# david-zwicker/video-analysis

Measured on AMD Instinct MI355X. Metric: frames/sec (bg-sub+blur+thresh+CCL) 1080p uint8, higher is better.
Workload: dtype u8; 1 GPU; cfg3_1080p_full_chain: 1920x1080 uint8, batch 256/GPU, running-mean bg-sub (f64 state) + sigma=5 Gaussian (q8.8) + threshold 20 + 5x5 dilate/erode + 4-connected labelling + object counts; inputs resident in HBM; engine=bg=1 gauss=mfma-i8(ksize=31) thresh=20 morph=2 ccl=4, video=one clip per rank, overlap=off, world_size=1, backend=single process

## Files before the change

### video-analysis_amd/csrc/va_api.hip

```cpp
#include <dlfcn.h>
#include <stdarg.h>
#include <stdlib.h>

#include <mutex>
#include <vector>
#include <new>

#include "va_common.h"

namespace va {

static thread_local char g_err[512] = "";

void set_error(const char *fmt, ...)
{
    va_list ap;
    va_start(ap, fmt);
    vsnprintf(g_err, sizeof(g_err), fmt, ap);
    va_end(ap);
}
const char *get_error() { return g_err; }

struct ScratchBlock {
    void *ptr;
// ... 108 lines not shown
    void *blur;
    void *gscratch;
    int planes_wp;
    uint32_t *bits[2][2];
    void *ccl_ws[2];
    size_t ccl_ws_bytes;
    size_t bits_bytes;
    bool overlap;
    int slot;
    hipStream_t side;
    int paint_grid;
    hipEvent_t ev_front;
    hipEvent_t ev_paint[2];
    bool paint_pending[2];
    const char *paint_lo[2], *paint_hi[2];
    const char *pstat_lo[2], *pstat_hi[2];
    int32_t *labels_scratch;
    int32_t *counts_scratch;
    TapsQ8 tq;
    TapsF32 tf;
    RowSpans se[VA_MAX_MORPH_OPS];
    bool fused;
    bool mfma;
    bool f32_fused;
    char desc[160];
    StageProfiler *prof;
};

template <class T>
static int resize_any(const T *src, T *dst, int n, int src_h, int src_w, int c, int dst_h, int dst_w,
                      int interpolation, void *stream, const char *who)
{
    VA_ENTER();
    VA_REQUIRE(src && dst && src != dst, "%s: src/dst must be distinct non-NULL", who);
    VA_REQUIRE(n >= 0 && src_h > 0 && src_w > 0 && dst_h > 0 && dst_w > 0 && c >= 1 && c <= 4,
               "%s: bad shape (%d,%d,%d,%d) -> (%d,%d)", who, n, src_h, src_w, c, dst_h, dst_w);
    VA_REQUIRE((size_t)src_h * src_w < kMaxFramePixels && (size_t)dst_h * dst_w < kMaxFramePixels,
               "%s: frames above 2^29 pixels are not supported", who);
    VA_REQUIRE(interpolation >= VA_INTER_NEAREST && interpolation <= VA_INTER_LANCZOS4,
               "%s: interpolation %d not supported (0 nearest, 1 linear, 2 cubic, 3 area, 4 lanczos4)", who,
               interpolation);
    ScratchLease scratch;
    int rc = scratch.acquire(resize_scratch_bytes(src_h, src_w, dst_h, dst_w), as_stream(stream));
    if (rc)
        return rc;
    if constexpr (sizeof(T) == 1)
// ... 954 lines not shown
    }
    for (int i = 0; i < cfg->morph_count; i++) {
        if (cfg->morph_op[i] != VA_MORPH_ERODE && cfg->morph_op[i] != VA_MORPH_DILATE) {
            set_error("va_pipeline_create: bad morph_op[%d]=%d", i, cfg->morph_op[i]);
            pipeline_free(p);
            return VA_ERR_INVALID;
        }
        PIPE_TRY(make_row_spans(cfg->morph_shape[i], cfg->morph_ksize[i], &p->se[i]));
    }
    if (cfg->bg_mode != VA_BG_NONE) {
        p->bg_bytes = p->px * (cfg->bg_mode == VA_BG_EMA ? sizeof(float) : sizeof(double));
        PIPE_MALLOC(p->bg_state, p->bg_bytes);
        if (p->f32_fused && cfg->bg_mode == VA_BG_EMA)
            PIPE_MALLOC(p->bg_state_alt, p->bg_bytes);
        p->bg_in_u8_range = true;
        hipError_t e = hipMemset(p->bg_state, 0, p->bg_bytes);
        if (e != hipSuccess) {
            set_error("va_pipeline_create: hipMemset failed: %s", hipGetErrorString(e));
            pipeline_free(p);
            return VA_ERR_HIP;
        }
        if (!p->f32_fused)
            PIPE_MALLOC(p->diff, nb * p->px * esz);
        if (cfg->bg_mode == VA_BG_MEAN)
            PIPE_MALLOC(p->bg_recip, bg_scratch_bytes(cfg->max_batch));
    }
    if (cfg->sigma > 0 && !p->fused) {
        size_t gs = cfg->dtype == VA_U8 ? gauss_generic_u8_scratch_bytes(nb * p->px, p->tq) : nb * p->px * 4;
        if (cfg->dtype == VA_U8) {
            p->planes_wp = planes_width(cfg->height, cfg->width, cfg->channels, p->tq);
            if (p->planes_wp)
                gs = planes_scratch_bytes(cfg->max_batch, cfg->height, p->planes_wp, cfg->channels);
        }
        PIPE_MALLOC(p->gscratch, gs);
        PIPE_MALLOC(p->blur, nb * p->px * esz);
    }
    if (masks) {
        size_t bb = align_up(nb * cfg->height * p->w32 * sizeof(uint32_t));
        p->bits_bytes = bb;
        PIPE_MALLOC(p->bits[0][0], bb);
        PIPE_MALLOC(p->bits[0][1], bb);
        if (cfg->connectivity) {
            p->ccl_ws_bytes = ccl_rows_workspace_bytes(cfg->max_batch, cfg->height);
            PIPE_MALLOC(p->ccl_ws[0], p->ccl_ws_bytes);
            PIPE_MALLOC(p->counts_scratch, align_up(nb * sizeof(int32_t)));
            PIPE_MALLOC(p->labels_scratch, nb * p->frame_px * sizeof(int32_t));
// ... 166 lines not shown
    VA_MARK(nullptr);

    if (c.dtype == VA_F32 && p->f32_fused) {
        VA_REQUIRE(reinterpret_cast<uintptr_t>(frames) % 16 == 0 &&
                       (!filtered_out || reinterpret_cast<uintptr_t>(filtered_out) % 16 == 0),
                   "va_pipeline_run: float32 pipelines need 16-byte aligned frames_dev / filtered_out_dev "
                   "(hipMalloc'ed buffers and whole-frame offsets into them are)");
        void *dst = filtered_out ? filtered_out : p->blur;
        const bool ema = c.bg_mode == VA_BG_EMA;
        rc = launch_gauss_f32_fused((const float *)frames, (float *)dst, (float *)p->gscratch,
                                    ema ? (const float *)p->bg_state : nullptr,
                                    ema ? (float *)p->bg_state_alt : nullptr, p->n_seen, (double)c.bg_rate, n,
                                    c.height, c.width, c.channels, p->tf, st, prof);
        if (rc)
            return rc;
        if (ema && n > 0) {
            std::swap(p->bg_state, p->bg_state_alt);
            p->n_seen += n;
        }
        return VA_OK;
    }
    if (c.bg_mode != VA_BG_NONE) {
        rc = launch_bg(c.bg_mode, c.dtype, cur, p->diff, p->bg_state, p->n_seen, (double)c.bg_rate,
                       n, p->px, st, p->bg_recip, p->bg_in_u8_range);
        if (rc)
            return rc;
        p->n_seen += n;
        cur = p->diff;
        VA_MARK("bg");
    }

    const bool want_ccl = masks && c.connectivity && (labels_out || counts_out || stats_out);
    const bool defer_paint = p->overlap && want_ccl && (labels_out != nullptr || stats_out != nullptr);
    const int slot = defer_paint ? p->slot : 0;
    if (p->overlap && p->paint_pending[slot])
        VA_HIP(hipStreamWaitEvent(st, p->ev_paint[slot], 0));
    uint32_t *const *bits = p->bits[slot];

    bool have_bits = false;
    if (c.sigma > 0) {
        if (c.dtype == VA_U8 && p->mfma && masks && mask_out && !filtered_out && c.morph_count == 0 && !want_ccl &&
            reinterpret_cast<uintptr_t>(mask_out) % 4 == 0) {
            rc = launch_gauss_mfma_u8((const uint8_t *)cur, mask_out, nullptr, c.thresh, n, c.height, c.width, p->tq,
                                      st, c.maxval);
            if (rc)
                return rc;
            VA_MARK("gauss_mfma_mask8");
            return VA_OK;
        }
        if (c.dtype == VA_U8 && p->fused) {
            if (p->mfma)
                rc = launch_gauss_mfma_u8((const uint8_t *)cur, (uint8_t *)filtered_out, masks ? bits[0] : nullptr,
                                          c.thresh, n, c.height, c.width, p->tq, st);
            else
                rc = launch_gauss_fused_u8((const uint8_t *)cur, (uint8_t *)filtered_out, masks ? bits[0] : nullptr,
                                           c.thresh, n, c.height, c.width, p->tq, st);
            if (rc)
                return rc;
            have_bits = masks;
            cur = filtered_out;
            VA_MARK(p->mfma ? "gauss_mfma" : "gauss_fused");
        } else {
            void *dst = filtered_out ? filtered_out : p->blur;
            if (c.dtype == VA_U8 && p->planes_wp)
                rc = blur_u8_planes((const uint8_t *)cur, (uint8_t *)dst, n, c.height, c.width,
                                    p->planes_wp, c.channels, p->tq, p->gscratch, st);
            else if (c.dtype == VA_U8)
                rc = launch_gauss_generic_u8((const uint8_t *)cur, (uint8_t *)dst,
                                             p->gscratch, n, c.height, c.width,
                                             c.channels, p->tq, st);
            else if (gauss_f32_fast_supported(c.width, c.channels, p->tf))
                rc = launch_gauss_f32_fast((const float *)cur, (float *)dst, (float *)p->gscratch, n,
                                           c.height, c.width, c.channels, p->tf, st);
            else
                rc = launch_gauss_generic_f32((const float *)cur, (float *)dst,
                                              (float *)p->gscratch, n, c.height, c.width,
// ... 255 lines not shown
```

### video-analysis_amd/csrc/va_common.h

```cpp
#pragma once
#include <hip/hip_runtime.h>
#include <stdint.h>
#include <stdio.h>
#include <string.h>

#include "../../include/videoanalysis_hip.h"

namespace va {

void set_error(const char *fmt, ...) __attribute__((format(printf, 1, 2)));
const char *get_error();

inline hipStream_t as_stream(void *s) { return reinterpret_cast<hipStream_t>(s); }

#define VA_HIP(call)                                                                        \
    do {                                                                                    \
        hipError_t _e = (call);                                                             \
        if (_e != hipSuccess) {                                                             \
            va::set_error("%s failed: %s (%s:%d)", #call, hipGetErrorString(_e), __FILE__,  \
                          __LINE__);                                                        \
            return _e == hipErrorOutOfMemory ? VA_ERR_NOMEM : VA_ERR_HIP;                   \
        }                                                                                   \
    } while (0)

// ... 65 lines not shown
int launch_gauss_generic_u8(const uint8_t *src, uint8_t *dst, void *scratch, int n, int h,
                            int w, int c, const TapsQ8 &taps, hipStream_t st);
int launch_gauss_generic_f32(const float *src, float *dst, float *scratch, int n, int h, int w,
                             int c, const TapsF32 &taps, hipStream_t st);
bool gauss_f32_fast_supported(int w, int c, const TapsF32 &taps);
int launch_gauss_f32_fast(const float *src, float *dst, float *scratch, int n, int h, int w, int c,
                          const TapsF32 &taps, hipStream_t st);
#if defined(__HIPCC__)
__device__ __forceinline__ void lds_barrier()
{
    asm volatile("s_waitcnt lgkmcnt(0)\n\ts_barrier" ::: "memory");
}
#endif
void gauss_f32_test_hook(int generic_columns);
bool gauss_f32_fused_supported(int h, int w, int c, const TapsF32 &taps);
int launch_gauss_f32_fused(const float *src, float *dst, float *scratch, const float *bg, float *bg_out,
                           int64_t n_seen, double rate, int n, int h, int w, int c, const TapsF32 &taps,
                           hipStream_t st, StageProfiler *prof = nullptr);
bool gauss_fused_supported(int w, int h, const TapsQ8 &taps);
int launch_gauss_fused_u8(const uint8_t *src, uint8_t *dst, uint32_t *bits, int thresh, int n,
                          int h, int w, const TapsQ8 &taps, hipStream_t st);
bool gauss_mfma_supported(int w, int h, const TapsQ8 &taps);
int launch_gauss_mfma_u8(const uint8_t *src, uint8_t *dst, uint32_t *bits, int thresh, int n,
                         int h, int w, const TapsQ8 &taps, hipStream_t st, int mask8_maxval = 0);

size_t bg_scratch_bytes(int n);
int launch_bg(int mode, int dtype, const void *frames, void *diff, void *state, int64_t n_seen,
              double rate, int n, size_t px, hipStream_t st, double *recip_scratch = nullptr,
              bool mean_in_u8_range = false);
int launch_welford(const uint8_t *frames, double *mean, double *m2, int64_t n_seen, int n,
                   size_t px, hipStream_t st);

int launch_temporal_stats(const void *frames, int dtype, double *mean, double *m2, int64_t n_seen, int n,
                          size_t px, hipStream_t st);
int launch_threshold_u8(const uint8_t *src, uint8_t *dst, size_t count, int thresh, int maxval,
                        hipStream_t st);
int launch_time_difference(const uint8_t *a, const uint8_t *b, int16_t *out, size_t count,
                           hipStream_t st);
int launch_mono_mean(const uint8_t *src, uint8_t *dst, size_t pixels, hipStream_t st);
bool launch_pointwise_u8_x4(const uint8_t *src, uint8_t *dst, size_t out_samples, int src_c, int mono, int normalize,
                            double fmin, double fmax, double alpha, double tmin, hipStream_t st);
int launch_channel_planes(const uint8_t *src, uint8_t *dst, int n, int h, int w, int wp, int c,
                          bool split, hipStream_t st);
int launch_rot90(const void *src, void *dst, int n, int h, int w, int elem_bytes, int k,
                 hipStream_t st);
int launch_normalize_u8(const uint8_t *src, uint8_t *dst, size_t count, double fmin, double fmax,
                        double alpha, double tmin, hipStream_t st);

int launch_pack_bits(const uint8_t *src, uint32_t *bits, int n, int h, int w, int thresh,
                     hipStream_t st);
int launch_unpack_bits(const uint32_t *bits, uint8_t *dst, int n, int h, int w, int maxval,
                       hipStream_t st);
// ... 94 lines not shown
```

### video-analysis_amd/csrc/va_gauss_mfma.hip

```cpp
#include "va_common.h"

namespace va {

namespace {

typedef int v4i __attribute__((ext_vector_type(4)));
typedef int v16i __attribute__((ext_vector_type(16)));
typedef uint32_t u4 __attribute__((ext_vector_type(4)));
typedef u4 u4_unaligned __attribute__((aligned(1)));

constexpr int kWaves = 4;
constexpr int kTileCols = kWaves * 32;
constexpr int kLdsStride = kTileCols + 32 + 16;
static_assert((kLdsStride / 16) % 2 == 1, "LDS row stride must be an odd multiple of 16 bytes");
constexpr int kTapTable = 128;
#ifndef GMF_DST_AUX
#define GMF_DST_AUX 0
#endif
constexpr int kFlushTiles = 8;
constexpr int kFlushRows = 32 * kFlushTiles;
static_assert(kFlushRows == kWaves * 64, "one thread per collected row at a flush");

struct MfmaTaps {
    int ksize;
    int sum;
    int8_t w[36];
};

__device__ __forceinline__ uint32_t bswap32(uint32_t v)
{
    return __builtin_amdgcn_perm(0u, v, 0x00010203u);
}

template <bool HAS_DST, bool HAS_BITS, bool MASK8 = false>
__global__ __launch_bounds__(kWaves * 64, 4) void gauss_mfma_kernel(
    const uint8_t *__restrict__ src, uint8_t *__restrict__ dst, uint32_t *__restrict__ bits,
    int thresh, int h, int w, int w32, int nstrips, int blocks_per_frame, int nframes, MfmaTaps tp,
    int maxval = 255)
{
    __shared__ __attribute__((aligned(16))) uint8_t s_stage[2][32 * kLdsStride];
    __shared__ int8_t s_taps[kTapTable];
    __shared__ __attribute__((aligned(16))) uint32_t s_bits[2][kFlushRows][kWaves];
    constexpr int kDstStride = kTileCols / 4 + 1;
    __shared__ uint32_t s_dst[HAS_DST ? 2 : 1][HAS_DST ? 32 : 1][kDstStride];

    if (threadIdx.x < kTapTable) {
        const int e = (int)threadIdx.x - 48;
        int v = 0;
#pragma unroll
        for (int k = 0; k < 33; k++)
            v = (e == k && k < tp.ksize) ? (int)tp.w[k] : v;
        s_taps[threadIdx.x] = (int8_t)v;
    }
    __syncthreads();

    const int xcd = blockIdx.x & 7, q = blockIdx.x >> 3;
    const int frame = (q / blocks_per_frame) * 8 + xcd;
    const int wave = threadIdx.x >> 6, lane = threadIdx.x & 63;
    const int strip = (q % blocks_per_frame) * kWaves + wave;
    if (frame >= nframes)
        return;
    const bool active = strip < nstrips;

// ... 70 lines not shown
            gb = mir_b ? rb : gb;
        }
        *reinterpret_cast<u4 *>(buf + row_a * kLdsStride + 16 * ch_a) = ga ^ 0x80808080u;
        if (wave == 0)
            *reinterpret_cast<u4 *>(buf + row_b * kLdsStride + 16 * ch_b) = gb ^ 0x80808080u;
    };

    v16i c_init;
#pragma unroll
    for (int i = 0; i < 16; i++)
        c_init[i] = c_lo;
    asm volatile("" : "+v"(c_init));

    const uint32_t kOob = 0xFFFFFFFFu;
    __amdgpu_buffer_rsrc_t bits_rsrc = __builtin_amdgcn_make_buffer_rsrc(
        HAS_BITS ? (void *)(bits + (size_t)frame * h * w32) : nullptr, 0, h * w32 * 4, 0x00027000);
    __amdgpu_buffer_rsrc_t dst_rsrc = __builtin_amdgcn_make_buffer_rsrc(
        HAS_DST ? (void *)(dst + (size_t)frame * h * w) : nullptr, 0, h * w, 0x00027000);
    const int xbw = xb >> 5;
    const int valid = max(0, min(32, w - x0));
    const uint32_t colmask = valid < 32 ? (1u << valid) - 1u : ~0u;
    const int frag_off = nn * kLdsStride + 32 * wave + 16 * hh;

    u4 ga, gb = {};
    fetch(0, ga, gb);
    stage_write(s_stage[0], ga, gb);
    fetch(1, ga, gb);
    __syncthreads();
    v4i prev_hi = {}, prev_lo = {};
    v16i yh = {}, yl = {};

    for (int t = 0; t <= ntiles + 1; t++) {
        const uint8_t *cur_buf = s_stage[t & 1];
        uint8_t *next_buf = s_stage[(t + 1) & 1];
        const v4i a0 = *reinterpret_cast<const v4i *>(cur_buf + frag_off);
        const v4i a1 = *reinterpret_cast<const v4i *>(cur_buf + frag_off + 32);
        v16i x = {};
        v4i vout = {};
        if (HAS_DST)
#pragma unroll
            for (int j = 0; j < 4; j++)
                vout[j] = (int)s_dst[(t + 1) & 1][tid >> 3][(tid & 7) * 4 + j];
        x = __builtin_amdgcn_mfma_i32_32x32x32_i8(a0, brow[0], x, 0, 0, 0);
        x = __builtin_amdgcn_mfma_i32_32x32x32_i8(a1, brow[1], x, 0, 0, 0);

        {
            uint32_t p = 0;
            int tv[16];
#pragma unroll
            for (int i = 15; i >= 0; i--) {
                tv[i] = (yh[i] << 8) + yl[i];
                if (HAS_BITS)
                    p = __builtin_amdgcn_alignbit(p, (uint32_t)tv[i], 31);
            }
            const int u = t - 2;
#ifndef GMF_NO_DST_LDS
            if (HAS_DST) {
#pragma unroll
                for (int g = 0; g < 4; g++) {
                    if (MASK8) {
                        const uint32_t t01 = __builtin_amdgcn_perm((uint32_t)tv[4 * g + 1], (uint32_t)tv[4 * g], 0x0c0c0703u);
                        const uint32_t t23 = __builtin_amdgcn_perm((uint32_t)tv[4 * g + 3], (uint32_t)tv[4 * g + 2], 0x07030c0cu);
                        s_dst[u & 1][nn][8 * wave + 2 * g + hh] = (t01 | t23) & (0x01010101u * (uint32_t)maxval);
                    } else {
                        const uint32_t d0 = (uint32_t)(k_dst - tv[4 * g]), d1 = (uint32_t)(k_dst - tv[4 * g + 1]);
                        const uint32_t d2 = (uint32_t)(k_dst - tv[4 * g + 2]), d3 = (uint32_t)(k_dst - tv[4 * g + 3]);
                        s_dst[u & 1][nn][8 * wave + 2 * g + hh] =
                            __builtin_amdgcn_perm(d1, d0, 0x0c0c0602u) | __builtin_amdgcn_perm(d3, d2, 0x06020c0cu);
                    }
                }
            }
#endif
            if (HAS_BITS) {
                uint32_t wd = (p & 0xFu) | ((p & 0xF0u) << 4) | ((p & 0xF00u) << 8) | ((p & 0xF000u) << 12);
                wd <<= 4 * hh;
                const auto sw = __builtin_amdgcn_permlane32_swap(wd, wd, false, false);
                if (hh == 0 && u >= 0)
                    s_bits[(u / kFlushTiles) & 1][(u % kFlushTiles) * 32 + nn][wave] =
                        active ? (wd | sw[1]) & colmask : 0u;
            }
        }

        stage_write(next_buf, ga, gb);
        fetch(min(t + 2, ntiles), ga, gb);
        if (HAS_DST) {
            const int us = t - 3, r = tid >> 3, c16 = (tid & 7) * 16, y = 32 * us + r;
#ifdef GMF_NO_DST_STORE
            const bool ok = false;
#else
            const bool ok = us >= 0 && y < h && xb + c16 < w;
#endif
            __builtin_amdgcn_raw_buffer_store_b128(vout, dst_rsrc, ok ? (uint32_t)(y * w + xb + c16) : kOob, 0, GMF_DST_AUX);
        }

        v4i cur_hi, cur_lo;
#pragma unroll
        for (int g = 0; g < 4; g++) {
            const uint32_t t01 = __builtin_amdgcn_perm((uint32_t)x[4 * g + 1], (uint32_t)x[4 * g], 0x05010400u);
            const uint32_t t23 = __builtin_amdgcn_perm((uint32_t)x[4 * g + 3], (uint32_t)x[4 * g + 2], 0x05010400u);
            cur_lo[g] = (int)(__builtin_amdgcn_perm(t23, t01, 0x05040100u) ^ 0x80808080u);
            cur_hi[g] = (int)__builtin_amdgcn_perm(t23, t01, 0x07060302u);
        }

        yh = __builtin_amdgcn_mfma_i32_32x32x32_i8(prev_hi, bcol[0], v16i{}, 0, 0, 0);
        yl = __builtin_amdgcn_mfma_i32_32x32x32_i8(prev_lo, bcol[0], c_init, 0, 0, 0);
        yh = __builtin_amdgcn_mfma_i32_32x32x32_i8(cur_hi, bcol[1], yh, 0, 0, 0);
        yl = __builtin_amdgcn_mfma_i32_32x32x32_i8(cur_lo, bcol[1], yl, 0, 0, 0);
        prev_hi = cur_hi;
        prev_lo = cur_lo;
        lds_barrier();

        const int u = t - 2;
        if (HAS_BITS && u >= 0 && (u % kFlushTiles == kFlushTiles - 1 || u == ntiles - 1)) {
            const int g = u / kFlushTiles, y = g * kFlushRows + tid;
            const bool ok = y < h && tid < (u % kFlushTiles + 1) * 32;
            const v4i v = *reinterpret_cast<const v4i *>(&s_bits[g & 1][tid][0]);
            const uint32_t off = (uint32_t)(y * w32 + xbw) * 4u;
            if (xbw + kWaves <= w32) {
                __builtin_amdgcn_raw_buffer_store_b128(v, bits_rsrc, ok ? off : kOob, 0, 0);
            } else {
#pragma unroll
                for (int k = 0; k < kWaves; k++)
                    __builtin_amdgcn_raw_buffer_store_b32(v[k], bits_rsrc,
                                                          ok && xbw + k < w32 ? off + 4 * k : kOob, 0, 0);
            }
        }
    }
    if (HAS_DST) {
        const int us = ntiles - 1, r = tid >> 3, c16 = (tid & 7) * 16, y = 32 * us + r;
        const bool ok = y < h && xb + c16 < w;
        v4i v;
#pragma unroll
        for (int j = 0; j < 4; j++)
            v[j] = (int)s_dst[us & 1][r][(tid & 7) * 4 + j];
        __builtin_amdgcn_raw_buffer_store_b128(v, dst_rsrc, ok ? (uint32_t)(y * w + xb + c16) : kOob, 0, 0);
    }
}

}

bool gauss_mfma_supported(int w, int h, const TapsQ8 &taps)
{
    if (w < 64 || h < 32 || (w % 16) != 0)
        return false;
    if (taps.ksize < 3 || taps.ksize / 2 > 16)
        return false;
    int sum = 0;
    for (int i = 0; i < taps.ksize; i++) {
        if (taps.t[i] > 127)
            return false;
        sum += taps.t[i];
    }
    return sum <= 256;
}

int launch_gauss_mfma_u8(const uint8_t *src, uint8_t *dst, uint32_t *bits, int thresh, int n,
                         int h, int w, const TapsQ8 &taps, hipStream_t st, int mask8_maxval)
{
    VA_REQUIRE(src && (dst || bits), "mfma gaussian: no output requested");
    VA_REQUIRE(mask8_maxval <= 0 || (dst && !bits && thresh >= 0 && mask8_maxval <= 255),
               "mfma gaussian: the byte-mask form writes dst only and needs a threshold");
    VA_REQUIRE(gauss_mfma_supported(w, h, taps), "mfma gaussian: unsupported kernel size %d",
               taps.ksize);
    VA_REQUIRE(reinterpret_cast<uintptr_t>(src) % 16 == 0 &&
                   (!dst || reinterpret_cast<uintptr_t>(dst) % 4 == 0),
               "mfma gaussian: the frame buffers must be 16-byte aligned");
    if (n == 0)
        return VA_OK;
    MfmaTaps tp = {};
    tp.ksize = taps.ksize;
    for (int i = 0; i < taps.ksize; i++) {
        tp.w[i] = (int8_t)taps.t[i];
        tp.sum += taps.t[i];
    }
    const int nstrips = cdiv(w, 32), w32 = words_per_row(w);
    const int bpf = cdiv(w, kTileCols);
    dim3 grid((unsigned)(8 * cdiv(n, 8) * bpf));
    if (mask8_maxval > 0)
        gauss_mfma_kernel<true, false, true><<<grid, kWaves * 64, 0, st>>>(src, dst, bits, thresh, h, w, w32, nstrips, bpf, n, tp,
                                                                            mask8_maxval);
    else if (dst && bits)
        gauss_mfma_kernel<true, true><<<grid, kWaves * 64, 0, st>>>(src, dst, bits, thresh, h, w, w32, nstrips, bpf, n, tp);
    else if (dst)
        gauss_mfma_kernel<true, false><<<grid, kWaves * 64, 0, st>>>(src, dst, bits, thresh, h, w, w32, nstrips, bpf, n, tp);
    else
        gauss_mfma_kernel<false, true><<<grid, kWaves * 64, 0, st>>>(src, dst, bits, thresh, h, w, w32, nstrips, bpf, n, tp);
    VA_LAUNCH_CHECK("gauss_mfma_kernel");
    return VA_OK;
}

}
```

### video-analysis_amd/csrc/va_point.hip

```cpp
#include <math.h>

#include "va_common.h"

namespace va {

namespace {

constexpr int kBlock = 256;
constexpr int kVec = 8;

__device__ __forceinline__ uint8_t sat_u8_trunc(double d)
{
    const int v = (int)d;
    return (uint8_t)(v > 255 ? 255 : v);
}

template <int V>
__global__ void __launch_bounds__(kBlock)
bg_mean_u8_kernel(const uint8_t *__restrict__ frames, uint8_t *__restrict__ diff,
                  double *__restrict__ mean, long long n_seen, int n, size_t px)
{
    size_t i0 = ((size_t)blockIdx.x * kBlock + threadIdx.x) * V;
    if (i0 >= px)
        return;
    double m[V];
#pragma unroll
    for (int k = 0; k < V; k++)
        m[k] = mean[i0 + k];
    for (int f = 0; f < n; f++) {
        uint8_t p[V];
        if (V == 8) {
            uint2 v = *reinterpret_cast<const uint2 *>(frames + (size_t)f * px + i0);
            memcpy(p, &v, 8);
        } else {
            p[0] = frames[(size_t)f * px + i0];
        }
        const double dn = (double)(n_seen + f), dn1 = (double)(n_seen + f + 1);
        uint8_t o[V];
#pragma unroll
        for (int k = 0; k < V; k++) {
            double fr = (double)p[k];
            o[k] = sat_u8_trunc(fabs(fr - m[k]));
            m[k] = m[k] * dn / dn1 + fr / dn1;
        }
        if (diff) {
            if (V == 8) {
                uint2 v;
                memcpy(&v, o, 8);
                *reinterpret_cast<uint2 *>(diff + (size_t)f * px + i0) = v;
            } else {
                diff[(size_t)f * px + i0] = o[0];
            }
        }
    }
#pragma unroll
    for (int k = 0; k < V; k++)
        mean[i0 + k] = m[k];
}

__device__ __forceinline__ double div_by_uniform(double x, double d, double y)
{
    const double q = x * y;
    const double r = fma(-q, d, x);
    return fma(r, y, q);
}

__global__ void __launch_bounds__(kBlock)
bg_reciprocals_kernel(double *__restrict__ y, long long n_seen, int n)
{
    const int f = blockIdx.x * kBlock + threadIdx.x;
    if (f < n)
        y[f] = 1.0 / (double)(n_seen + f + 1);
}

struct RecipArgs {
    double r[256];
    double lo[256];
    __device__ double operator[](int f) const { return r[f]; }
};
__device__ __forceinline__ double clear_low9(double y)
{
    return __builtin_bit_cast(double, __builtin_bit_cast(unsigned long long, y) & ~0x1FFull);
}

template <int V, typename RECIP, bool BOUNDED, bool SPLIT = false>
__global__ void __launch_bounds__(kBlock)
bg_mean_u8_fast_kernel(const uint8_t *__restrict__ frames, uint8_t *__restrict__ diff,
                       double *__restrict__ mean, const RECIP recip, long long n_seen, int n, size_t px)
{
    size_t i0 = ((size_t)blockIdx.x * kBlock + threadIdx.x) * V;
    if (i0 >= px)
        return;
    double m[V];
#pragma unroll
    for (int k = 0; k < V; k++)
        m[k] = mean[i0 + k];
    typedef unsigned int v2u __attribute__((ext_vector_type(V / 4)));
    constexpr int kAhead = 8;
    const uint8_t *src = frames + i0;
    v2u cur[kAhead], nxt[kAhead];
#pragma unroll
    for (int j = 0; j < kAhead; j++)
        nxt[j] = __builtin_nontemporal_load(
            reinterpret_cast<const v2u *>(src + (size_t)min(j, n - 1) * px));
    for (int f0 = 0; f0 < n; f0 += kAhead) {
#pragma unroll
        for (int j = 0; j < kAhead; j++)
            cur[j] = nxt[j];
        if (f0 + kAhead < n) {
#pragma unroll
            for (int j = 0; j < kAhead; j++)
                nxt[j] = __builtin_nontemporal_load(reinterpret_cast<const v2u *>(
                    src + (size_t)min(f0 + kAhead + j, n - 1) * px));
        }
// ... 5 lines not shown
            uint8_t p[V], o[V];
            memcpy(p, &cur[j], V);
            const double dn = (double)(n_seen + f), dn1 = (double)(n_seen + f + 1);
            const double y = recip[f];
            double yh = 0.0, yl = 0.0;
            if constexpr (SPLIT) {
                yh = clear_low9(y);
                yl = recip.lo[f];
            }
#pragma unroll
            for (int k = 0; k < V; k++) {
                const double fr = (double)p[k];
                o[k] = BOUNDED ? (uint8_t)(int)fabs(fr - m[k]) : sat_u8_trunc(fabs(fr - m[k]));
                double q2;
                if constexpr (SPLIT)
                    q2 = fma(fr, yl, fr * yh);
                else
                    q2 = div_by_uniform(fr, dn1, y);
                m[k] = div_by_uniform(m[k] * dn, dn1, y) + q2;
            }
            if (diff) {
                v2u v;
                memcpy(&v, o, V);
                __builtin_nontemporal_store(v, reinterpret_cast<v2u *>(diff + (size_t)f * px + i0));
            }
        }
    }
#pragma unroll
    for (int k = 0; k < V; k++)
        mean[i0 + k] = m[k];
}

template <int V>
__global__ void __launch_bounds__(kBlock)
bg_static_u8_kernel(const uint8_t *__restrict__ frames, uint8_t *__restrict__ diff,
                    const double *__restrict__ bg, int n, size_t px)
{
    size_t i0 = ((size_t)blockIdx.x * kBlock + threadIdx.x) * V;
    if (i0 >= px)
        return;
    double m[V];
#pragma unroll
    for (int k = 0; k < V; k++)
        m[k] = bg[i0 + k];
    for (int f = 0; f < n; f++) {
        uint8_t p[V], o[V];
        if (V == 8) {
            uint2 v = *reinterpret_cast<const uint2 *>(frames + (size_t)f * px + i0);
            memcpy(p, &v, 8);
        } else {
            p[0] = frames[(size_t)f * px + i0];
        }
#pragma unroll
        for (int k = 0; k < V; k++)
            o[k] = sat_u8_trunc(fabs((double)p[k] - m[k]));
        if (V == 8) {
            uint2 v;
            memcpy(&v, o, 8);
            *reinterpret_cast<uint2 *>(diff + (size_t)f * px + i0) = v;
        } else {
            diff[(size_t)f * px + i0] = o[0];
        }
    }
}

template <int V>
__global__ void __launch_bounds__(kBlock)
bg_ema_u8_kernel(const uint8_t *__restrict__ frames, uint8_t *__restrict__ diff,
                 float *__restrict__ bg, long long n_seen, float rate, int n, size_t px)
{
    size_t i0 = ((size_t)blockIdx.x * kBlock + threadIdx.x) * V;
    if (i0 >= px)
        return;
    float m[V];
#pragma unroll
    for (int k = 0; k < V; k++)
        m[k] = bg[i0 + k];
    for (int f = 0; f < n; f++) {
        uint8_t p[V], o[V];
        if (V == 8) {
            uint2 v = *reinterpret_cast<const uint2 *>(frames + (size_t)f * px + i0);
            memcpy(p, &v, 8);
        } else {
            p[0] = frames[(size_t)f * px + i0];
        }
        const bool first = (n_seen + f) == 0;
#pragma unroll
        for (int k = 0; k < V; k++) {
            float fr = (float)p[k];
            if (first)
                m[k] = fr;
            float d = fr - m[k];
            float a = truncf(fabsf(d));
            o[k] = (uint8_t)(int)(a > 255.0f ? 255.0f : a);
            float step = rate * d;
            m[k] = m[k] + step;
        }
        if (diff) {
            if (V == 8) {
                uint2 v;
                memcpy(&v, o, 8);
                *reinterpret_cast<uint2 *>(diff + (size_t)f * px + i0) = v;
            } else {
                diff[(size_t)f * px + i0] = o[0];
            }
        }
    }
#pragma unroll
    for (int k = 0; k < V; k++)
        bg[i0 + k] = m[k];
}

template <int V>
__global__ void __launch_bounds__(kBlock)
bg_ema_f32_kernel(const float *__restrict__ frames, float *__restrict__ diff,
                  float *__restrict__ bg, long long n_seen, float rate, int n, size_t px)
{
    size_t i0 = ((size_t)blockIdx.x * kBlock + threadIdx.x) * V;
    if (i0 >= px)
        return;
    float m[V];
#pragma unroll
    for (int k = 0; k < V; k++)
        m[k] = bg[i0 + k];
    for (int f = 0; f < n; f++) {
        float p[V], o[V];
        if (V == 4) {
// ... 158 lines not shown
}

__global__ void __launch_bounds__(kBlock)
normalize_u8_kernel(const uint8_t *__restrict__ src, uint8_t *__restrict__ dst, size_t count,
                    double fmin, double fmax, double alpha, double tmin)
{
    size_t i = (size_t)blockIdx.x * kBlock + threadIdx.x;
    if (i >= count)
        return;
    double f = (double)src[i];
    f = f < fmin ? fmin : (f > fmax ? fmax : f);
    double v = (f - fmin) * alpha + tmin;
    int iv = (int)v;
    dst[i] = (uint8_t)iv;
}

inline bool aligned(const void *p, size_t a) { return (reinterpret_cast<uintptr_t>(p) % a) == 0; }

}

size_t bg_scratch_bytes(int n) { return sizeof(double) * (size_t)(n > 0 ? n : 1); }

int launch_bg(int mode, int dtype, const void *frames, void *diff, void *state, int64_t n_seen,
              double rate, int n, size_t px, hipStream_t st, double *recip_scratch, bool mean_in_u8_range)
{
    VA_REQUIRE(frames && state, "va_bg_update: frames/state must not be NULL");
    VA_REQUIRE(n >= 0 && px > 0, "va_bg_update: bad sizes n=%d px=%zu", n, px);
    if (n == 0)
        return VA_OK;
    if (dtype == VA_U8) {
        const uint8_t *fr = (const uint8_t *)frames;
        uint8_t *df = (uint8_t *)diff;
        bool vec = (px % kVec == 0) && aligned(fr, 8) && (!df || aligned(df, 8));
        int grid = vec ? cdiv((long long)(px / kVec), kBlock) : cdiv((long long)px, kBlock);
        if (mode == VA_BG_MEAN) {
            const bool wide = px % 16 == 0 && aligned(fr, 16) && (!df || aligned(df, 16));
            if (vec && n <= 256) {
                RecipArgs ra;
                for (int f = 0; f < 256; f++) {
                    const double d = (double)(n_seen + (f < n ? f : 0) + 1), y = 1.0 / d;
                    unsigned long long bits;
                    memcpy(&bits, &y, 8);
                    bits &= ~0x1FFull;
                    double yh;
                    memcpy(&yh, &bits, 8);
                    ra.r[f] = y;
                    ra.lo[f] = fma(y, fma(-d, y, 1.0), y - yh);
                }
#ifdef BG_NO_SPLIT
                const bool split = false;
#else
                const bool split = n_seen + n < (1ll << 40);
#endif
                if (wide && mean_in_u8_range && split)
                    bg_mean_u8_fast_kernel<16, RecipArgs, true, true><<<cdiv((long long)(px / 16), kBlock), kBlock, 0, st>>>(
                        fr, df, (double *)state, ra, n_seen, n, px);
                else if (wide && mean_in_u8_range)
                    bg_mean_u8_fast_kernel<16, RecipArgs, true><<<cdiv((long long)(px / 16), kBlock), kBlock, 0, st>>>(
                        fr, df, (double *)state, ra, n_seen, n, px);
                else if (wide && split)
                    bg_mean_u8_fast_kernel<16, RecipArgs, false, true><<<cdiv((long long)(px / 16), kBlock), kBlock, 0, st>>>(
                        fr, df, (double *)state, ra, n_seen, n, px);
                else if (wide)
                    bg_mean_u8_fast_kernel<16, RecipArgs, false><<<cdiv((long long)(px / 16), kBlock), kBlock, 0, st>>>(
                        fr, df, (double *)state, ra, n_seen, n, px);
                else
                    bg_mean_u8_fast_kernel<8, RecipArgs, false><<<grid, kBlock, 0, st>>>(fr, df, (double *)state, ra,
                                                                                        n_seen, n, px);
            } else if (vec && recip_scratch) {
                bg_reciprocals_kernel<<<cdiv(n, kBlock), kBlock, 0, st>>>(recip_scratch, n_seen, n);
                VA_LAUNCH_CHECK("bg_reciprocals_kernel");
                if (wide)
                    bg_mean_u8_fast_kernel<16, const double *, false><<<cdiv((long long)(px / 16), kBlock), kBlock, 0, st>>>(
                        fr, df, (double *)state, recip_scratch, n_seen, n, px);
                else
                    bg_mean_u8_fast_kernel<8, const double *, false><<<grid, kBlock, 0, st>>>(
                        fr, df, (double *)state, recip_scratch, n_seen, n, px);
            } else if (vec)
                bg_mean_u8_kernel<8><<<grid, kBlock, 0, st>>>(fr, df, (double *)state, n_seen, n, px);
            else
                bg_mean_u8_kernel<1><<<grid, kBlock, 0, st>>>(fr, df, (double *)state, n_seen, n, px);
        } else if (mode == VA_BG_EMA) {
            if (vec)
                bg_ema_u8_kernel<8><<<grid, kBlock, 0, st>>>(fr, df, (float *)state, n_seen,
                                                            (float)rate, n, px);
            else
                bg_ema_u8_kernel<1><<<grid, kBlock, 0, st>>>(fr, df, (float *)state, n_seen,
                                                            (float)rate, n, px);
        } else if (mode == VA_BG_STATIC) {
            VA_REQUIRE(df, "va_bg_update: static mode needs diff_out");
            if (vec)
                bg_static_u8_kernel<8><<<grid, kBlock, 0, st>>>(fr, df, (const double *)state, n, px);
            else
                bg_static_u8_kernel<1><<<grid, kBlock, 0, st>>>(fr, df, (const double *)state, n, px);
        } else {
            VA_REQUIRE(false, "va_bg_update: unsupported mode %d for u8 frames", mode);
        }
    } else if (dtype == VA_F32) {
        VA_REQUIRE(mode == VA_BG_EMA, "va_bg_update: float32 frames support VA_BG_EMA only");
        const float *fr = (const float *)frames;
        float *df = (float *)diff;
        bool vec = (px % 4 == 0) && aligned(fr, 16) && (!df || aligned(df, 16));
        int grid = vec ? cdiv((long long)(px / 4), kBlock) : cdiv((long long)px, kBlock);
        if (vec)
            bg_ema_f32_kernel<4><<<grid, kBlock, 0, st>>>(fr, df, (float *)state, n_seen,
                                                         (float)rate, n, px);
        else
            bg_ema_f32_kernel<1><<<grid, kBlock, 0, st>>>(fr, df, (float *)state, n_seen,
                                                         (float)rate, n, px);
    } else {
        VA_REQUIRE(false, "va_bg_update: unknown dtype %d", dtype);
    }
    VA_LAUNCH_CHECK("bg kernel");
    return VA_OK;
}

int launch_welford(const uint8_t *frames, double *mean, double *m2, int64_t n_seen, int n,
// ... 289 lines not shown
```

Measured before the change: 311,900 frames/s.

## Write bg-sub difference frames in 16-column blocks for direct MFMA blur loads

The background-subtraction kernels now write difference frames in a column-block layout (16-byte-wide columns stored contiguously down the frame) whenever the MFMA Gaussian path is enabled. The MFMA blur kernel gains a COLBLK variant that loads its operand fragments straight from global memory with buffer loads into a register ring. This skips the LDS staging double buffer and most per-tile barriers, and it handles image edges with lane swaps and byte reversal. In exchange the bg kernels use a strided, less coalesced write pattern, and the edge-reflection logic adds complexity and correctness risk.

```diff
diff --git a/video-analysis_amd/csrc/va_api.hip b/video-analysis_amd/csrc/va_api.hip
--- a/video-analysis_amd/csrc/va_api.hip
+++ b/video-analysis_amd/csrc/va_api.hip
@@ -154,6 +154,7 @@
     RowSpans se[VA_MAX_MORPH_OPS];
     bool fused;
     bool mfma;
+    bool diff_colblocks;
     bool f32_fused;
     char desc[160];
     StageProfiler *prof;
@@ -1154,6 +1155,9 @@
         }
         if (!p->f32_fused)
             PIPE_MALLOC(p->diff, nb * p->px * esz);
+#ifndef VA_DIFF_ROWMAJOR
+        p->diff_colblocks = p->mfma;
+#endif
         if (cfg->bg_mode == VA_BG_MEAN)
             PIPE_MALLOC(p->bg_recip, bg_scratch_bytes(cfg->max_batch));
     }
@@ -1366,7 +1370,7 @@
     }
     if (c.bg_mode != VA_BG_NONE) {
         rc = launch_bg(c.bg_mode, c.dtype, cur, p->diff, p->bg_state, p->n_seen, (double)c.bg_rate,
-                       n, p->px, st, p->bg_recip, p->bg_in_u8_range);
+                       n, p->px, st, p->bg_recip, p->bg_in_u8_range, p->diff_colblocks ? c.width : 0);
         if (rc)
             return rc;
         p->n_seen += n;
@@ -1386,7 +1390,7 @@
         if (c.dtype == VA_U8 && p->mfma && masks && mask_out && !filtered_out && c.morph_count == 0 && !want_ccl &&
             reinterpret_cast<uintptr_t>(mask_out) % 4 == 0) {
             rc = launch_gauss_mfma_u8((const uint8_t *)cur, mask_out, nullptr, c.thresh, n, c.height, c.width, p->tq,
-                                      st, c.maxval);
+                                      st, c.maxval, cur == p->diff && p->diff_colblocks);
             if (rc)
                 return rc;
             VA_MARK("gauss_mfma_mask8");
@@ -1395,7 +1399,8 @@
         if (c.dtype == VA_U8 && p->fused) {
             if (p->mfma)
                 rc = launch_gauss_mfma_u8((const uint8_t *)cur, (uint8_t *)filtered_out, masks ? bits[0] : nullptr,
-                                          c.thresh, n, c.height, c.width, p->tq, st);
+                                          c.thresh, n, c.height, c.width, p->tq, st, 0,
+                                          cur == p->diff && p->diff_colblocks);
             else
                 rc = launch_gauss_fused_u8((const uint8_t *)cur, (uint8_t *)filtered_out, masks ? bits[0] : nullptr,
                                            c.thresh, n, c.height, c.width, p->tq, st);
diff --git a/video-analysis_amd/csrc/va_common.h b/video-analysis_amd/csrc/va_common.h
--- a/video-analysis_amd/csrc/va_common.h
+++ b/video-analysis_amd/csrc/va_common.h
@@ -111,12 +111,13 @@
                           int h, int w, const TapsQ8 &taps, hipStream_t st);
 bool gauss_mfma_supported(int w, int h, const TapsQ8 &taps);
 int launch_gauss_mfma_u8(const uint8_t *src, uint8_t *dst, uint32_t *bits, int thresh, int n,
-                         int h, int w, const TapsQ8 &taps, hipStream_t st, int mask8_maxval = 0);
+                         int h, int w, const TapsQ8 &taps, hipStream_t st, int mask8_maxval = 0,
+                         bool src_colblocks = false);
 
 size_t bg_scratch_bytes(int n);
 int launch_bg(int mode, int dtype, const void *frames, void *diff, void *state, int64_t n_seen,
               double rate, int n, size_t px, hipStream_t st, double *recip_scratch = nullptr,
-              bool mean_in_u8_range = false);
+              bool mean_in_u8_range = false, int diff_colblock_w = 0);
 int launch_welford(const uint8_t *frames, double *mean, double *m2, int64_t n_seen, int n,
                    size_t px, hipStream_t st);
 
diff --git a/video-analysis_amd/csrc/va_gauss_mfma.hip b/video-analysis_amd/csrc/va_gauss_mfma.hip
--- a/video-analysis_amd/csrc/va_gauss_mfma.hip
+++ b/video-analysis_amd/csrc/va_gauss_mfma.hip
@@ -1,3 +1,5 @@
+#include <type_traits>
+
 #include "va_common.h"
 
 namespace va {
@@ -20,6 +22,12 @@
 constexpr int kFlushTiles = 8;
 constexpr int kFlushRows = 32 * kFlushTiles;
 static_assert(kFlushRows == kWaves * 64, "one thread per collected row at a flush");
+#ifndef GMF_RING
+#define GMF_RING 1
+#endif
+#ifndef GMF_RING_DST
+#define GMF_RING_DST GMF_RING
+#endif
 
 struct MfmaTaps {
     int ksize;
@@ -32,13 +40,26 @@
     return __builtin_amdgcn_perm(0u, v, 0x00010203u);
 }
 
-template <bool HAS_DST, bool HAS_BITS, bool MASK8 = false>
+template <int S>
+__device__ __forceinline__ v4i reverse16(v4i lo, v4i hi)
+{
+    const uint32_t c[8] = {(uint32_t)lo.x, (uint32_t)lo.y, (uint32_t)lo.z, (uint32_t)lo.w,
+                           (uint32_t)hi.x, (uint32_t)hi.y, (uint32_t)hi.z, (uint32_t)hi.w};
+    constexpr int q = S >> 2, r = S & 3;
+    uint32_t d[4];
+#pragma unroll
+    for (int k = 0; k < 4; k++)
+        d[k] = __builtin_amdgcn_alignbyte(c[k + q + 1], c[k + q], r);
+    return v4i{(int)bswap32(d[3]), (int)bswap32(d[2]), (int)bswap32(d[1]), (int)bswap32(d[0])};
+}
+
+template <bool HAS_DST, bool HAS_BITS, bool MASK8 = false, bool COLBLK = false>
 __global__ __launch_bounds__(kWaves * 64, 4) void gauss_mfma_kernel(
     const uint8_t *__restrict__ src, uint8_t *__restrict__ dst, uint32_t *__restrict__ bits,
     int thresh, int h, int w, int w32, int nstrips, int blocks_per_frame, int nframes, MfmaTaps tp,
     int maxval = 255)
 {
-    __shared__ __attribute__((aligned(16))) uint8_t s_stage[2][32 * kLdsStride];
+    __shared__ __attribute__((aligned(16))) uint8_t s_stage[COLBLK ? 1 : 2][COLBLK ? 16 : 32 * kLdsStride];
     __shared__ int8_t s_taps[kTapTable];
     __shared__ __attribute__((aligned(16))) uint32_t s_bits[2][kFlushRows][kWaves];
     constexpr int kDstStride = kTileCols / 4 + 1;
@@ -155,19 +176,10 @@
     const uint32_t colmask = valid < 32 ? (1u << valid) - 1u : ~0u;
     const int frag_off = nn * kLdsStride + 32 * wave + 16 * hh;
 
-    u4 ga, gb = {};
-    fetch(0, ga, gb);
-    stage_write(s_stage[0], ga, gb);
-    fetch(1, ga, gb);
-    __syncthreads();
     v4i prev_hi = {}, prev_lo = {};
     v16i yh = {}, yl = {};
 
-    for (int t = 0; t <= ntiles + 1; t++) {
-        const uint8_t *cur_buf = s_stage[t & 1];
-        uint8_t *next_buf = s_stage[(t + 1) & 1];
-        const v4i a0 = *reinterpret_cast<const v4i *>(cur_buf + frag_off);
-        const v4i a1 = *reinterpret_cast<const v4i *>(cur_buf + frag_off + 32);
+    auto step = [&](const int t, const v4i a0, const v4i a1, auto &&refill) {
         v16i x = {};
         v4i vout = {};
         if (HAS_DST)
@@ -214,8 +226,7 @@
             }
         }
 
-        stage_write(next_buf, ga, gb);
-        fetch(min(t + 2, ntiles), ga, gb);
+        refill();
         if (HAS_DST) {
             const int us = t - 3, r = tid >> 3, c16 = (tid & 7) * 16, y = 32 * us + r;
 #ifdef GMF_NO_DST_STORE
@@ -241,10 +252,13 @@
         yl = __builtin_amdgcn_mfma_i32_32x32x32_i8(cur_lo, bcol[1], yl, 0, 0, 0);
         prev_hi = cur_hi;
         prev_lo = cur_lo;
-        lds_barrier();
+        if (!COLBLK || HAS_DST)
+            lds_barrier();
 
         const int u = t - 2;
         if (HAS_BITS && u >= 0 && (u % kFlushTiles == kFlushTiles - 1 || u == ntiles - 1)) {
+            if (COLBLK && !HAS_DST)
+                lds_barrier();
             const int g = u / kFlushTiles, y = g * kFlushRows + tid;
             const bool ok = y < h && tid < (u % kFlushTiles + 1) * 32;
             const v4i v = *reinterpret_cast<const v4i *>(&s_bits[g & 1][tid][0]);
@@ -258,6 +272,81 @@
                                                           ok && xbw + k < w32 ? off + 4 * k : kOob, 0, 0);
             }
         }
+    };
+
+    if constexpr (!COLBLK) {
+        u4 ga, gb = {};
+        fetch(0, ga, gb);
+        stage_write(s_stage[0], ga, gb);
+        fetch(1, ga, gb);
+        __syncthreads();
+        for (int t = 0; t <= ntiles + 1; t++) {
+            const uint8_t *cur_buf = s_stage[t & 1];
+            const v4i a0 = *reinterpret_cast<const v4i *>(cur_buf + frag_off);
+            const v4i a1 = *reinterpret_cast<const v4i *>(cur_buf + frag_off + 32);
+            step(t, a0, a1, [&] {
+                stage_write(s_stage[(t + 1) & 1], ga, gb);
+                fetch(min(t + 2, ntiles), ga, gb);
+            });
+        }
+    } else {
+        const int nb = w >> 4, cb = x0 >> 4;
+        const uint32_t colh = (uint32_t)h * 16;
+        const uint32_t off0 = (uint32_t)min(max(cb - 1 + hh, 0), nb - 1) * colh + 16u * nn;
+        const uint32_t off1 = (uint32_t)min(cb + 1 + hh, nb - 1) * colh + 16u * nn;
+        const __amdgpu_buffer_rsrc_t src_rsrc =
+            __builtin_amdgcn_make_buffer_rsrc((void *)fsrc, 0, h * w, 0x00027000);
+        auto load = [&](int t, v4i &a0, v4i &a1) {
+            if (t >= 1 && 32 * t + 16 <= h) {
+                const int so = (32 * t - 16) * 16;
+                a0 = __builtin_amdgcn_raw_buffer_load_b128(src_rsrc, off0, so, 0);
+                a1 = __builtin_amdgcn_raw_buffer_load_b128(src_rsrc, off1, so, 0);
+            } else {
+                const uint32_t dy = (uint32_t)(row_of(t, nn) - nn) * 16u;
+                a0 = __builtin_amdgcn_raw_buffer_load_b128(src_rsrc, off0 + dy, 0, 0);
+                a1 = __builtin_amdgcn_raw_buffer_load_b128(src_rsrc, off1 + dy, 0, 0);
+            }
+        };
+        const int cbu = __builtin_amdgcn_readfirstlane(cb);
+        const bool sel_l = cbu == 0 && hh == 0;
+        const bool sel_r1 = nb - cbu == 1 && hh == 0;
+        const bool sel_r2 = nb - cbu == 2 && hh == 1;
+
+        auto march = [&](auto edge) {
+            constexpr int kRing = HAS_DST ? GMF_RING_DST : GMF_RING;
+            v4i r0[kRing], r1[kRing];
+#pragma unroll
+            for (int j = 0; j < kRing; j++)
+                load(min(j, ntiles), r0[j], r1[j]);
+            for (int t0 = 0; t0 <= ntiles + 1; t0 += kRing) {
+#pragma unroll
+                for (int j = 0; j < kRing; j++) {
+                    const int t = t0 + j;
+                    if (t > ntiles + 1)
+                        break;
+                    v4i a0 = r0[j], a1 = r1[j];
+                    if constexpr (decltype(edge)::value) {
+                        v4i up0, dn1;
+#pragma unroll
+                        for (int k = 0; k < 4; k++) {
+                            const auto sw = __builtin_amdgcn_permlane32_swap((uint32_t)a0[k], (uint32_t)a1[k], false, false);
+                            dn1[k] = (int)sw[0];
+                            up0[k] = (int)sw[1];
+                        }
+                        const v4i ml = reverse16<1>(up0, a1), mr1 = reverse16<15>(a0, up0), mr2 = reverse16<15>(a0, dn1);
+                        a0 = sel_l ? ml : a0;
+                        a1 = sel_r1 ? mr1 : (sel_r2 ? mr2 : a1);
+                    }
+                    a0 ^= (int)0x80808080u;
+                    a1 ^= (int)0x80808080u;
+                    step(t, a0, a1, [&] { load(min(t + kRing, ntiles), r0[j], r1[j]); });
+                }
+            }
+        };
+        if (cbu == 0 || nb - cbu == 1 || nb - cbu == 2)
+            march(std::true_type{});
+        else
+            march(std::false_type{});
     }
     if (HAS_DST) {
         const int us = ntiles - 1, r = tid >> 3, c16 = (tid & 7) * 16, y = 32 * us + r;
@@ -288,7 +377,7 @@
 }
 
 int launch_gauss_mfma_u8(const uint8_t *src, uint8_t *dst, uint32_t *bits, int thresh, int n,
-                         int h, int w, const TapsQ8 &taps, hipStream_t st, int mask8_maxval)
+                         int h, int w, const TapsQ8 &taps, hipStream_t st, int mask8_maxval, bool src_colblocks)
 {
     VA_REQUIRE(src && (dst || bits), "mfma gaussian: no output requested");
     VA_REQUIRE(mask8_maxval <= 0 || (dst && !bits && thresh >= 0 && mask8_maxval <= 255),
@@ -309,15 +398,22 @@
     const int nstrips = cdiv(w, 32), w32 = words_per_row(w);
     const int bpf = cdiv(w, kTileCols);
     dim3 grid((unsigned)(8 * cdiv(n, 8) * bpf));
-    if (mask8_maxval > 0)
-        gauss_mfma_kernel<true, false, true><<<grid, kWaves * 64, 0, st>>>(src, dst, bits, thresh, h, w, w32, nstrips, bpf, n, tp,
-                                                                            mask8_maxval);
-    else if (dst && bits)
-        gauss_mfma_kernel<true, true><<<grid, kWaves * 64, 0, st>>>(src, dst, bits, thresh, h, w, w32, nstrips, bpf, n, tp);
-    else if (dst)
-        gauss_mfma_kernel<true, false><<<grid, kWaves * 64, 0, st>>>(src, dst, bits, thresh, h, w, w32, nstrips, bpf, n, tp);
+    auto run = [&](auto colblk) {
+        constexpr bool CB = decltype(colblk)::value;
+        if (mask8_maxval > 0)
+            gauss_mfma_kernel<true, false, true, CB><<<grid, kWaves * 64, 0, st>>>(src, dst, bits, thresh, h, w, w32, nstrips,
+                                                                                bpf, n, tp, mask8_maxval);
+        else if (dst && bits)
+            gauss_mfma_kernel<true, true, false, CB><<<grid, kWaves * 64, 0, st>>>(src, dst, bits, thresh, h, w, w32, nstrips, bpf, n, tp);
+        else if (dst)
+            gauss_mfma_kernel<true, false, false, CB><<<grid, kWaves * 64, 0, st>>>(src, dst, bits, thresh, h, w, w32, nstrips, bpf, n, tp);
+        else
+            gauss_mfma_kernel<false, true, false, CB><<<grid, kWaves * 64, 0, st>>>(src, dst, bits, thresh, h, w, w32, nstrips, bpf, n, tp);
+    };
+    if (src_colblocks)
+        run(std::true_type{});
     else
-        gauss_mfma_kernel<false, true><<<grid, kWaves * 64, 0, st>>>(src, dst, bits, thresh, h, w, w32, nstrips, bpf, n, tp);
+        run(std::false_type{});
     VA_LAUNCH_CHECK("gauss_mfma_kernel");
     return VA_OK;
 }
diff --git a/video-analysis_amd/csrc/va_point.hip b/video-analysis_amd/csrc/va_point.hip
--- a/video-analysis_amd/csrc/va_point.hip
+++ b/video-analysis_amd/csrc/va_point.hip
@@ -9,6 +9,31 @@
 constexpr int kBlock = 256;
 constexpr int kVec = 8;
 
+struct DiffLayout {
+    int h = 0, w = 0;
+    static size_t threads(int V, size_t px, int h, int w)
+    {
+        return h > 0 ? (size_t)cdiv(w, 128) * h * (128 / V) : (px + V - 1) / V;
+    }
+    template <int V>
+    __device__ __forceinline__ bool map(uint32_t g, size_t px, size_t &src, size_t &dst) const
+    {
+        if (h == 0) {
+            src = dst = (size_t)g * V;
+            return src < px;
+        }
+        constexpr uint32_t kPerRow = 128 / V;
+        const uint32_t per_group = (uint32_t)h * kPerRow;
+        const uint32_t cg = g / per_group, rem = g - cg * per_group;
+        const int row = (int)(rem / kPerRow), col = (int)(cg * 128 + (rem % kPerRow) * V);
+        if (col >= w)
+            return false;
+        src = (size_t)row * w + col;
+        dst = (size_t)(col >> 4) * h * 16 + (size_t)row * 16 + (col & 15);
+        return true;
+    }
+};
+
 __device__ __forceinline__ uint8_t sat_u8_trunc(double d)
 {
     const int v = (int)d;
@@ -18,10 +43,10 @@
 template <int V>
 __global__ void __launch_bounds__(kBlock)
 bg_mean_u8_kernel(const uint8_t *__restrict__ frames, uint8_t *__restrict__ diff,
-                  double *__restrict__ mean, long long n_seen, int n, size_t px)
-{
-    size_t i0 = ((size_t)blockIdx.x * kBlock + threadIdx.x) * V;
-    if (i0 >= px)
+                  double *__restrict__ mean, long long n_seen, int n, size_t px, DiffLayout lay)
+{
+    size_t i0, o0;
+    if (!lay.template map<V>(blockIdx.x * kBlock + threadIdx.x, px, i0, o0))
         return;
     double m[V];
 #pragma unroll
@@ -47,9 +72,9 @@
             if (V == 8) {
                 uint2 v;
                 memcpy(&v, o, 8);
-                *reinterpret_cast<uint2 *>(diff + (size_t)f * px + i0) = v;
+                *reinterpret_cast<uint2 *>(diff + (size_t)f * px + o0) = v;
             } else {
-                diff[(size_t)f * px + i0] = o[0];
+                diff[(size_t)f * px + o0] = o[0];
             }
         }
     }
@@ -86,10 +111,10 @@
 template <int V, typename RECIP, bool BOUNDED, bool SPLIT = false>
 __global__ void __launch_bounds__(kBlock)
 bg_mean_u8_fast_kernel(const uint8_t *__restrict__ frames, uint8_t *__restrict__ diff,
-                       double *__restrict__ mean, const RECIP recip, long long n_seen, int n, size_t px)
-{
-    size_t i0 = ((size_t)blockIdx.x * kBlock + threadIdx.x) * V;
-    if (i0 >= px)
+                       double *__restrict__ mean, const RECIP recip, long long n_seen, int n, size_t px, DiffLayout lay)
+{
+    size_t i0, o0;
+    if (!lay.template map<V>(blockIdx.x * kBlock + threadIdx.x, px, i0, o0))
         return;
     double m[V];
 #pragma unroll
@@ -141,7 +166,7 @@
             if (diff) {
                 v2u v;
                 memcpy(&v, o, V);
-                __builtin_nontemporal_store(v, reinterpret_cast<v2u *>(diff + (size_t)f * px + i0));
+                __builtin_nontemporal_store(v, reinterpret_cast<v2u *>(diff + (size_t)f * px + o0));
             }
         }
     }
@@ -153,10 +178,10 @@
 template <int V>
 __global__ void __launch_bounds__(kBlock)
 bg_static_u8_kernel(const uint8_t *__restrict__ frames, uint8_t *__restrict__ diff,
-                    const double *__restrict__ bg, int n, size_t px)
-{
-    size_t i0 = ((size_t)blockIdx.x * kBlock + threadIdx.x) * V;
-    if (i0 >= px)
+                    const double *__restrict__ bg, int n, size_t px, DiffLayout lay)
+{
+    size_t i0, o0;
+    if (!lay.template map<V>(blockIdx.x * kBlock + threadIdx.x, px, i0, o0))
         return;
     double m[V];
 #pragma unroll
@@ -176,9 +201,9 @@
         if (V == 8) {
             uint2 v;
             memcpy(&v, o, 8);
-            *reinterpret_cast<uint2 *>(diff + (size_t)f * px + i0) = v;
-        } else {
-            diff[(size_t)f * px + i0] = o[0];
+            *reinterpret_cast<uint2 *>(diff + (size_t)f * px + o0) = v;
+        } else {
+            diff[(size_t)f * px + o0] = o[0];
         }
     }
 }
@@ -186,10 +211,10 @@
 template <int V>
 __global__ void __launch_bounds__(kBlock)
 bg_ema_u8_kernel(const uint8_t *__restrict__ frames, uint8_t *__restrict__ diff,
-                 float *__restrict__ bg, long long n_seen, float rate, int n, size_t px)
-{
-    size_t i0 = ((size_t)blockIdx.x * kBlock + threadIdx.x) * V;
-    if (i0 >= px)
+                 float *__restrict__ bg, long long n_seen, float rate, int n, size_t px, DiffLayout lay)
+{
+    size_t i0, o0;
+    if (!lay.template map<V>(blockIdx.x * kBlock + threadIdx.x, px, i0, o0))
         return;
     float m[V];
 #pragma unroll
@@ -219,9 +244,9 @@
             if (V == 8) {
                 uint2 v;
                 memcpy(&v, o, 8);
-                *reinterpret_cast<uint2 *>(diff + (size_t)f * px + i0) = v;
+                *reinterpret_cast<uint2 *>(diff + (size_t)f * px + o0) = v;
             } else {
-                diff[(size_t)f * px + i0] = o[0];
+                diff[(size_t)f * px + o0] = o[0];
             }
         }
     }
@@ -426,19 +451,30 @@
 size_t bg_scratch_bytes(int n) { return sizeof(double) * (size_t)(n > 0 ? n : 1); }
 
 int launch_bg(int mode, int dtype, const void *frames, void *diff, void *state, int64_t n_seen,
-              double rate, int n, size_t px, hipStream_t st, double *recip_scratch, bool mean_in_u8_range)
+              double rate, int n, size_t px, hipStream_t st, double *recip_scratch, bool mean_in_u8_range,
+              int diff_colblock_w)
 {
     VA_REQUIRE(frames && state, "va_bg_update: frames/state must not be NULL");
     VA_REQUIRE(n >= 0 && px > 0, "va_bg_update: bad sizes n=%d px=%zu", n, px);
+    VA_REQUIRE(diff_colblock_w == 0 || (dtype == VA_U8 && diff && diff_colblock_w % 16 == 0 &&
+                                        px % (size_t)diff_colblock_w == 0),
+               "va_bg_update: column-block differences need u8 frames, diff_out and a width divisible by 16");
     if (n == 0)
         return VA_OK;
     if (dtype == VA_U8) {
         const uint8_t *fr = (const uint8_t *)frames;
         uint8_t *df = (uint8_t *)diff;
+        DiffLayout lay;
+        if (diff_colblock_w > 0) {
+            lay.w = diff_colblock_w;
+            lay.h = (int)(px / (size_t)diff_colblock_w);
+        }
+        auto grid_of = [&](int v) { return cdiv((long long)DiffLayout::threads(v, px, lay.h, lay.w), kBlock); };
         bool vec = (px % kVec == 0) && aligned(fr, 8) && (!df || aligned(df, 8));
-        int grid = vec ? cdiv((long long)(px / kVec), kBlock) : cdiv((long long)px, kBlock);
+        int grid = vec ? grid_of(kVec) : grid_of(1);
         if (mode == VA_BG_MEAN) {
             const bool wide = px % 16 == 0 && aligned(fr, 16) && (!df || aligned(df, 16));
+            const int grid16 = grid_of(16);
             if (vec && n <= 256) {
                 RecipArgs ra;
                 for (int f = 0; f < 256; f++) {
@@ -457,46 +493,46 @@
                 const bool split = n_seen + n < (1ll << 40);
 #endif
                 if (wide && mean_in_u8_range && split)
-                    bg_mean_u8_fast_kernel<16, RecipArgs, true, true><<<cdiv((long long)(px / 16), kBlock), kBlock, 0, st>>>(
-                        fr, df, (double *)state, ra, n_seen, n, px);
+                    bg_mean_u8_fast_kernel<16, RecipArgs, true, true><<<grid16, kBlock, 0, st>>>(
+                        fr, df, (double *)state, ra, n_seen, n, px, lay);
                 else if (wide && mean_in_u8_range)
-                    bg_mean_u8_fast_kernel<16, RecipArgs, true><<<cdiv((long long)(px / 16), kBlock), kBlock, 0, st>>>(
-                        fr, df, (double *)state, ra, n_seen, n, px);
+                    bg_mean_u8_fast_kernel<16, RecipArgs, true><<<grid16, kBlock, 0, st>>>(
+                        fr, df, (double *)state, ra, n_seen, n, px, lay);
                 else if (wide && split)
-                    bg_mean_u8_fast_kernel<16, RecipArgs, false, true><<<cdiv((long long)(px / 16), kBlock), kBlock, 0, st>>>(
-                        fr, df, (double *)state, ra, n_seen, n, px);
+                    bg_mean_u8_fast_kernel<16, RecipArgs, false, true><<<grid16, kBlock, 0, st>>>(
+                        fr, df, (double *)state, ra, n_seen, n, px, lay);
                 else if (wide)
-                    bg_mean_u8_fast_kernel<16, RecipArgs, false><<<cdiv((long long)(px / 16), kBlock), kBlock, 0, st>>>(
-                        fr, df, (double *)state, ra, n_seen, n, px);
+                    bg_mean_u8_fast_kernel<16, RecipArgs, false><<<grid16, kBlock, 0, st>>>(
+                        fr, df, (double *)state, ra, n_seen, n, px, lay);
                 else
                     bg_mean_u8_fast_kernel<8, RecipArgs, false><<<grid, kBlock, 0, st>>>(fr, df, (double *)state, ra,
-                                                                                        n_seen, n, px);
+                                                                                        n_seen, n, px, lay);
             } else if (vec && recip_scratch) {
                 bg_reciprocals_kernel<<<cdiv(n, kBlock), kBlock, 0, st>>>(recip_scratch, n_seen, n);
                 VA_LAUNCH_CHECK("bg_reciprocals_kernel");
                 if (wide)
-                    bg_mean_u8_fast_kernel<16, const double *, false><<<cdiv((long long)(px / 16), kBlock), kBlock, 0, st>>>(
-                        fr, df, (double *)state, recip_scratch, n_seen, n, px);
+                    bg_mean_u8_fast_kernel<16, const double *, false><<<grid16, kBlock, 0, st>>>(
+                        fr, df, (double *)state, recip_scratch, n_seen, n, px, lay);
                 else
                     bg_mean_u8_fast_kernel<8, const double *, false><<<grid, kBlock, 0, st>>>(
-                        fr, df, (double *)state, recip_scratch, n_seen, n, px);
+                        fr, df, (double *)state, recip_scratch, n_seen, n, px, lay);
             } else if (vec)
-                bg_mean_u8_kernel<8><<<grid, kBlock, 0, st>>>(fr, df, (double *)state, n_seen, n, px);
+                bg_mean_u8_kernel<8><<<grid, kBlock, 0, st>>>(fr, df, (double *)state, n_seen, n, px, lay);
             else
-                bg_mean_u8_kernel<1><<<grid, kBlock, 0, st>>>(fr, df, (double *)state, n_seen, n, px);
+                bg_mean_u8_kernel<1><<<grid, kBlock, 0, st>>>(fr, df, (double *)state, n_seen, n, px, lay);
         } else if (mode == VA_BG_EMA) {
             if (vec)
                 bg_ema_u8_kernel<8><<<grid, kBlock, 0, st>>>(fr, df, (float *)state, n_seen,
-                                                            (float)rate, n, px);
+                                                            (float)rate, n, px, lay);
             else
                 bg_ema_u8_kernel<1><<<grid, kBlock, 0, st>>>(fr, df, (float *)state, n_seen,
-                                                            (float)rate, n, px);
+                                                            (float)rate, n, px, lay);
         } else if (mode == VA_BG_STATIC) {
             VA_REQUIRE(df, "va_bg_update: static mode needs diff_out");
             if (vec)
-                bg_static_u8_kernel<8><<<grid, kBlock, 0, st>>>(fr, df, (const double *)state, n, px);
+                bg_static_u8_kernel<8><<<grid, kBlock, 0, st>>>(fr, df, (const double *)state, n, px, lay);
             else
-                bg_static_u8_kernel<1><<<grid, kBlock, 0, st>>>(fr, df, (const double *)state, n, px);
+                bg_static_u8_kernel<1><<<grid, kBlock, 0, st>>>(fr, df, (const double *)state, n, px, lay);
         } else {
             VA_REQUIRE(false, "va_bg_update: unsupported mode %d for u8 frames", mode);
         }
```

Result: faster. 315,100 frames/s (median of 6 runs) (+1.0%).
